# seceq/zkir

Hardware: AMD Instinct MI355X
Metric: trace rows/sec (2^20-cycle fib: execution-trace fill + BabyBear NTT/LDE + Poseidon2 Merkle commitment) (higher is better)
Workload: dtype u32 (Baby Bear, 31-bit modular) / u64 trace words

## Files before the change

include/zkir_amd_experimental.h:

```cpp
#ifndef ZKIR_AMD_EXPERIMENTAL_H
#define ZKIR_AMD_EXPERIMENTAL_H
#include "zkir_amd.h"
#ifdef __cplusplus
extern "C" {
#endif

double zkir_modmul_peak_per_s(void* hip_stream);
double zkir_hbm_copy_peak_gbs(uint64_t bytes, void* hip_stream);
int zkir_commit_fused01_launch(const zkir_stark_ctx* ctx, const zkir_trace_columns* trace, uint64_t n_real, uint32_t* m, uint32_t width, uint32_t* out, void* hip_stream);
int zkir_ntt_strided_variant_launch(const zkir_stark_ctx* ctx, uint32_t* data, uint32_t width, int variant, int forward, void* hip_stream);

int zkir_commit_overlapped_launch(const zkir_stark_ctx* ctx, uint32_t* in, uint32_t width, uint32_t* out, uint32_t* tree, uint32_t group, void* hip_stream);

int zkir_lowdeg_prove_stages(zkir_stark_ctx* ctx, const uint32_t* lde_mat, uint32_t width, const uint32_t* tree, uint32_t num_queries, uint32_t pow_bits, uint32_t* proof_host,
                             uint64_t cap_words, uint64_t* n_words, float stage_ms[4], void* hip_stream);
int zkir_lowdeg_combine_launch(const zkir_stark_ctx* ctx, const uint32_t* lde_mat, uint32_t width, const uint32_t gamma[4], uint32_t* gpow_scratch, uint32_t* cw, void* hip_stream);

int zkir_eval_prove_stages(zkir_stark_ctx* ctx, const uint32_t* lde_mat, uint32_t width, const uint32_t* tree, const uint32_t* points, uint32_t n_points, uint32_t num_queries,
                           uint32_t pow_bits, uint32_t* proof_host, uint64_t cap_words, uint64_t* n_words, float stage_ms[6], void* hip_stream);
uint64_t zkir_eval_at_scratch_words(uint32_t log_n, uint32_t width, uint32_t n_points);
int zkir_eval_at_launch(const zkir_stark_ctx* ctx, const uint32_t* lde_mat, uint32_t width, const uint32_t* points, uint32_t n_points, uint32_t* scratch, uint32_t* evals, void* hip_stream);
uint64_t zkir_eval_quotient_scratch_words(uint32_t log_m, uint32_t width, uint32_t n_points);
int zkir_eval_quotient_launch(const zkir_stark_ctx* ctx, const uint32_t* lde_mat, uint32_t width, const uint32_t gamma[4], const uint32_t* points, uint32_t n_points,
                              const uint32_t* evals, uint32_t* scratch, uint32_t* cw, void* hip_stream);
// ... 26 lines not shown
int zkir_verify_many_memory_probe(const uint32_t* const* proofs, const uint64_t* proof_words, const zkir_public_inputs* const* expects, uint32_t n, int32_t* verdicts, uint32_t what,
                                  uint32_t index, int device, void* hip_stream);
int zkir_verify_many_tapes_host(const uint32_t* const* proofs, const uint64_t* proof_words, const zkir_public_inputs* const* expects, uint32_t n, int32_t* verdicts);
int zkir_verify_rate_many_tapes_host(const uint32_t* const* proofs, const uint64_t* proof_words, const zkir_public_inputs* const* expects, const uint32_t* min_queries,
                                     const uint32_t* min_pow_bits, uint32_t n, int32_t* verdicts);
int zkir_tape_sections_stage_host(const uint32_t* const* hash_secs, const uint64_t* hash_words, const uint32_t* const* wide_secs, const uint64_t* wide_words, const uint64_t* n_real,
                                  const uint64_t* code_end, const uint32_t* alphas, const uint32_t* lambdas, uint32_t n, int32_t* hash_verdicts, int32_t* wide_verdicts, uint32_t* digests,
                                  uint32_t* sums);
int zkir_tape_sections_stage_launch(const uint32_t* const* hash_secs, const uint64_t* hash_words, const uint32_t* const* wide_secs, const uint64_t* wide_words, const uint64_t* n_real,
                                    const uint64_t* code_end, const uint32_t* alphas, const uint32_t* lambdas, uint32_t n, int32_t* hash_verdicts, int32_t* wide_verdicts, uint32_t* digests,
                                    uint32_t* sums, void* hip_stream);
int zkir_verify_many_tapes_probe(const uint32_t* const* proofs, const uint64_t* proof_words, const zkir_public_inputs* const* expects, uint32_t n, int32_t* verdicts, uint32_t what,
                                 uint32_t index, int device, void* hip_stream);
void zkir_poseidon2_scaled_quads(const uint32_t* in, uint64_t n, uint32_t* full, uint32_t* quads);
int zkir_poseidon2_sponge_full_blocks(const uint32_t* words, uint32_t n_words, uint32_t form, uint32_t digest[4]);

#ifdef __cplusplus
}
#endif
#endif
```

zkir_amd/csrc/host.h:

```cpp
#pragma once

#include <sys/mman.h>

#include <atomic>
#include <cstdint>
#include <cstdlib>
#include <cstring>
#include <new>
#include <string>
#include <utility>
#include <vector>

#include "../../include/zkir_amd.h"

#define ZKIR_DEFAULT_TILE_ROWS 1024u

namespace zkir {

struct Status {
  int code = ZKIR_OK;
  std::string msg;
  bool ok() const { return code == ZKIR_OK; }
};

// ... 142 lines not shown
                         void* hip_stream);

struct LdeTables {
  int log_n;
  const uint32_t* tw_inv;
  const uint32_t* tw_fwd;
  const uint32_t* g_lo;
  const uint32_t* g_hi;
  const uint32_t* small_inv;
  const uint32_t* small_fwd;
  int log_blowup = 1;
  uint32_t* zero_slot = nullptr;
  uint32_t zero_epoch = 0;
};
constexpr uint32_t ZERO_FLAG_BLOCKS = 64;
void lde_run(const LdeTables& t, uint32_t* in, uint32_t n_blocks, uint32_t* out, void* hip_stream);
bool strided_variant_run(const LdeTables& t, uint32_t* data, uint32_t n_blocks, int variant, bool dit, void* hip_stream);
bool lde_run_fused01(const LdeTables& t, const zkir_trace_columns* trace, uint64_t n_real, uint32_t* in, uint32_t n_blocks, uint32_t* out, void* hip_stream);
}
```

zkir_amd/csrc/ntt.hip:

```cpp
#include <hip/hip_runtime.h>

#include <atomic>
#include <cstdlib>
#include <mutex>
#include <type_traits>

#include "../../include/zkir_amd.h"
#include "../../include/zkir_amd_experimental.h"
#include "babybear.h"
#include "host.h"

namespace {

constexpr int NT = 256;
__device__ __forceinline__ uint32_t bitrev(uint32_t x, int bits) { return bits == 0 ? 0u : __brev(x) >> (32 - bits); }

template <int K, int N, class F>
__device__ __forceinline__ void static_for(F&& f) {
  if constexpr (K < N) { f(std::integral_constant<int, K>{}); static_for<K + 1, N>(f); }
}

using u32x4 = uint32_t __attribute__((ext_vector_type(4)));
__device__ __forceinline__ u32x4 ld4(const uint4* p) { return *reinterpret_cast<const u32x4*>(p); }
__device__ __forceinline__ void st4(uint4* p, u32x4 v) { *reinterpret_cast<u32x4*>(p) = v; }

__device__ __forceinline__ void wave_sync_lds() { asm volatile("s_waitcnt lgkmcnt(0)" ::: "memory"); }

struct WTw { int32_t w, n; };
__device__ __forceinline__ WTw wtw(int32_t w) { return WTw{w, -w}; }
__device__ __forceinline__ void dit4w4(uint4& x0, uint4& x1, uint4& x2, uint4& x3, WTw w1, WTw w2, WTw w2i) {
#define ZKIR_Q(c, e) { int32_t a[4] = {(int32_t)x0.c, (int32_t)x1.c, (int32_t)x2.c, (int32_t)x3.c}, b[4] = {(int32_t)x0.e, (int32_t)x1.e, (int32_t)x2.e, (int32_t)x3.e}; \
                       bb::dit4w2(a, b, w1.w, w1.n, w2.w, w2.n, w2i.w, w2i.n); \
                       x0.c = (uint32_t)a[0]; x1.c = (uint32_t)a[1]; x2.c = (uint32_t)a[2]; x3.c = (uint32_t)a[3]; x0.e = (uint32_t)b[0]; x1.e = (uint32_t)b[1]; x2.e = (uint32_t)b[2]; x3.e = (uint32_t)b[3]; }
  ZKIR_Q(x, y) __builtin_amdgcn_sched_barrier(0); ZKIR_Q(z, w)
#undef ZKIR_Q
// ... 50 lines not shown
      const uint64_t v = q.t.registers[o];
      const int bits = q.t.reg_state[o] ? 30 : 20;
      const uint64_t mask = (1ull << bits) - 1;
      out[0] = (uint32_t)(v & mask); out[1] = (uint32_t)((v >> bits) & mask); out[2] = (uint32_t)(v >> (2 * bits));
    };
    uint32_t a[3], b[3];
    if (half == 0) { limbs(1, a); r.x = q.t.instruction[src] >> 19; r.y = a[0]; r.z = a[1]; r.w = a[2]; }
    else { limbs(2, a); limbs(3, b); r.x = a[0]; r.y = a[1]; r.z = a[2]; r.w = b[0]; }
  }
  return r;
}

template <bool DIT, int R, int C, int NTH, bool FUSED = false>
__global__ __launch_bounds__(NTH) void ntt_strided_r4_kernel(uint4* __restrict__ data, uint64_t blk_u4, uint32_t tiles_per_block, uint32_t total, int L, int s0,
                                                              const uint32_t* __restrict__ tw, const uint32_t* __restrict__ small, int log_small, uint32_t j4_m, int canon, TraceSrc01 fsrc = TraceSrc01{},
                                                              uint32_t* zflags = nullptr, uint32_t epoch = 0, int produce = 0) {
  constexpr int B = 2 * R;
  constexpr uint32_t POS = 1u << (B + C), QUADS = POS / 4, CMASK = (1u << C) - 1, PLANE = POS + 4;
  constexpr uint32_t MOVES = 2 * POS / NTH;
  static_assert(QUADS % NTH == 0 && NTH % (1 << C) == 0 && (2 * POS) % NTH == 0, "tile / thread geometry");
  extern __shared__ uint4 lds4[];
  const uint32_t n = 1u << L;
  const uint32_t stride_mid = DIT ? (1u << s0) : (n >> (s0 + B));
  const uint32_t lo_tiles = stride_mid >> C;
  auto geometry = [&](uint32_t w, uint4*& x, uint32_t& base, uint32_t& lo0, uint32_t& hi) {
    const uint32_t tile = w % tiles_per_block;
    x = data + (uint64_t)(w / tiles_per_block) * blk_u4;
    hi = tile / lo_tiles;
    lo0 = (tile % lo_tiles) << C;
    base = (DIT ? (hi << (s0 + B)) : hi * (n >> s0)) + lo0;
  };
  static_assert(QUADS == NTH, "one quad per lane and round");
  u32x4 pre[MOVES];
  uint4* x; uint32_t base, lo0, hi;
  uint64_t live = ~0ull;
  if (zflags && !produce) { const uint32_t l = threadIdx.x & 63; live = __ballot(l < total / tiles_per_block && zflags[l] == epoch); }
  auto next_live = [&](uint32_t ww) { while (ww < total && !((live >> (ww / tiles_per_block)) & 1)) ww += gridDim.x; return ww; };
  uint32_t w = next_live(blockIdx.x);
  if (w >= total) return;
  uint32_t sm[R];
#pragma unroll
  for (int r = 0; r < R; r++) {
    const int b = 2 * r;
    const uint32_t qq = threadIdx.x >> C;
    if (!DIT) sm[r] = small[bitrev(qq >> (B - 2 - b), b) << (log_small - (b + 2))];
    else sm[r] = small[(qq & ((1u << b) - 1)) << (log_small - (b + 2))];
  }
  const bool unit = s0 == 0;
  uint32_t tf_next[R] = {};
  auto tile_factors = [&](uint32_t hi_t) {
    if (DIT || unit) return;
    const uint32_t e = bitrev(hi_t, s0);
#pragma unroll
    for (int r = 0; r < R; r++) tf_next[r] = tw[e << (L - s0 - 2 * r - 2)];
// ... 2 lines not shown
  static_for<0, (int)MOVES>([&](auto kc) {
    constexpr uint32_t k = decltype(kc)::value;
    const uint32_t e = threadIdx.x + k * NTH, row = e >> (C + 1), wv = e & ((2u << C) - 1);
    if constexpr (FUSED) pre[k] = trace_quad01(fsrc, w / tiles_per_block, wv & 1, (uint64_t)base + (uint64_t)row * stride_mid + (wv >> 1));
    else pre[k] = ld4(&x[((uint64_t)base + (uint64_t)row * stride_mid) * 2 + wv]);
  });
  uint32_t tw_cur = 0;
  if (DIT) tw_cur = tw[(lo0 + (threadIdx.x & CMASK)) << (L - s0 - B)];
  tile_factors(hi);
  for (;;) {
    uint32_t nz = 0;
    static_for<0, (int)MOVES>([&](auto kc) {
      constexpr uint32_t k = decltype(kc)::value;
      const uint32_t e = threadIdx.x + k * NTH, row = e >> (C + 1), wv = e & ((2u << C) - 1);
      st4(&lds4[(wv & 1) * PLANE + ((row << C) | (wv >> 1))], pre[k]);
      if (produce) nz |= (pre[k].x | pre[k].y) | (pre[k].z | pre[k].w);
    });
    uint32_t tp[R];
    if (DIT) {
      uint32_t u = tw_cur;
#pragma unroll
      for (int r = R - 1; r >= 0; r--) { tp[r] = u; u = bb::mont_mul(u, u); u = bb::mont_mul(u, u); }
    } else {
#pragma unroll
      for (int r = 0; r < R; r++) tp[r] = tf_next[r];
    }
    bool dense = true;
    if (produce) {
      dense = __syncthreads_or(nz != 0) != 0;
      if (dense && threadIdx.x == 0) zflags[w / tiles_per_block] = epoch;
    } else {
      __syncthreads();
    }
    const uint32_t wn = next_live(w + gridDim.x);
    uint4* xn = x; uint32_t base_n = base, lo0_n = lo0, hi_n = hi;
    if (wn < total) {
      geometry(wn, xn, base_n, lo0_n, hi_n);
      static_for<0, (int)MOVES>([&](auto kc) {
        constexpr uint32_t k = decltype(kc)::value;
        const uint32_t e = threadIdx.x + k * NTH, row = e >> (C + 1), wv = e & ((2u << C) - 1);
        if constexpr (FUSED) pre[k] = trace_quad01(fsrc, wn / tiles_per_block, wv & 1, (uint64_t)base_n + (uint64_t)row * stride_mid + (wv >> 1));
        else pre[k] = ld4(&xn[((uint64_t)base_n + (uint64_t)row * stride_mid) * 2 + wv]);
      });
      if (DIT) tw_cur = tw[(lo0_n + (threadIdx.x & CMASK)) << (L - s0 - B)];
      tile_factors(hi_n);
// ... 27 lines not shown
          const WTw w2 = wtw(bb::mont_mul_centred(tp[r], sm[r]));
          const uint32_t w2u = bb::wcanon(w2.w);
          const WTw w1 = wtw(bb::mont_mul_centred(w2u, w2u)), w2i = wtw(bb::mont_mul_centred(w2u, j4_m));
          uint4 x0 = pl0[i0], x1 = pl0[i0 + d], x2 = pl0[i0 + 2 * d], x3 = pl0[i0 + 3 * d];
          dit4w4(x0, x1, x2, x3, w1, w2, w2i);
          pl0[i0] = x0; pl0[i0 + d] = x1; pl0[i0 + 2 * d] = x2; pl0[i0 + 3 * d] = x3;
          __builtin_amdgcn_sched_barrier(0);
          uint4 y0 = pl1[i0], y1 = pl1[i0 + d], y2 = pl1[i0 + 2 * d], y3 = pl1[i0 + 3 * d];
          dit4w4(y0, y1, y2, y3, w1, w2, w2i);
          pl1[i0] = y0; pl1[i0 + d] = y1; pl1[i0 + 2 * d] = y2; pl1[i0 + 3 * d] = y3;
        }
      }
      const bool wave_local = !DIT ? (r + 1 < R && B - 2 - b <= 6 - C) : (r + 1 < R && b + 2 <= 6 - C);
      if (wave_local) wave_sync_lds(); else __syncthreads();
    }
#pragma unroll
    for (uint32_t k = 0; k < MOVES; k++) {
      const uint32_t e = threadIdx.x + k * NTH, row = e >> (C + 1), wv = e & ((2u << C) - 1);
      uint4 v = lds4[(wv & 1) * PLANE + ((row << C) | (wv >> 1))];
      if (DIT && canon) v = canon4(v);
      x[((uint64_t)base + (uint64_t)row * stride_mid) * 2 + wv] = v;
    }
    }
    if (wn >= total) break;
    w = wn; x = xn; base = base_n; lo0 = lo0_n; hi = hi_n;
  }
}

template <bool DIT, int S>
__global__ __launch_bounds__(NT) void ntt_reg_kernel(uint4* __restrict__ data, uint64_t blk_u4, int L, int s0, const uint32_t* __restrict__ tw, uint32_t r4_m, uint32_t r8_m,
                                                       uint32_t r8_3_m, int canon) {
  constexpr int E = 1 << S;
  const uint32_t n = 1u << L;
  uint4* x = data + (uint64_t)blockIdx.y * blk_u4;
  const uint64_t item = (uint64_t)blockIdx.x * NT + threadIdx.x;
  if (item >= ((uint64_t)n >> S) * 2) return;
// ... 40 lines not shown
}

inline unsigned cu_count() {
  static std::mutex mu;
  static unsigned cached[64] = {};
  int dev = 0;
  if (hipGetDevice(&dev) != hipSuccess || dev < 0 || dev >= 64) return 256u;
  std::lock_guard<std::mutex> lk(mu);
  if (!cached[dev]) { hipDeviceProp_t p; cached[dev] = hipGetDeviceProperties(&p, dev) == hipSuccess && p.multiProcessorCount > 0 ? (unsigned)p.multiProcessorCount : 256u; }
  return cached[dev];
}
inline int persist() { static const int v = getenv("ZKIR_NTT_PERSIST") ? atoi(getenv("ZKIR_NTT_PERSIST")) : 1; return v; }

template <bool DIT, int R, int C, int NTH, bool FUSED = false>
void launch_strided_r4(uint32_t* data, uint64_t n, uint32_t n_blocks, int L, int s0, const uint32_t* tw, const uint32_t* small, int log_small, uint32_t j4_m, hipStream_t s,
                       const TraceSrc01* fsrc = nullptr, int canon = 0, uint32_t* zflags = nullptr, uint32_t epoch = 0, int produce = 0) {
  constexpr size_t lds = 16u * 2 * ((1u << (2 * R + C)) + 4);
  auto k = ntt_strided_r4_kernel<DIT, R, C, NTH, FUSED>;
  static std::atomic<uint64_t> attr_done{0};
  int dev = 0; (void)hipGetDevice(&dev);
  const uint64_t bit = 1ull << (dev & 63);
  if (!(attr_done.load(std::memory_order_relaxed) & bit)) { (void)hipFuncSetAttribute(reinterpret_cast<const void*>(k), hipFuncAttributeMaxDynamicSharedMemorySize, (int)lds); attr_done.fetch_or(bit); }
  const uint32_t tiles = (uint32_t)(n >> (2 * R + C)), total = tiles * n_blocks;
  const unsigned per_cu = (unsigned)((160u << 10) / lds) > 0 ? (unsigned)((160u << 10) / lds) : 1u;
  unsigned grid = persist() ? cu_count() * (per_cu > 8 ? 8 : per_cu) : total;
  if (grid > total) grid = total;
  hipLaunchKernelGGL(k, dim3(grid), dim3(NTH), lds, s, (uint4*)data, 2 * n, tiles, total, L, s0, tw, small, log_small, j4_m, canon, fsrc ? *fsrc : TraceSrc01{}, zflags, epoch, produce);
}

inline int strided_c() { static const int c = getenv("ZKIR_NTT_C") ? atoi(getenv("ZKIR_NTT_C")) : 2; return c; }

template <bool DIT>
uint32_t* run_strided_stages(uint32_t* data, uint64_t n, uint32_t n_blocks, int L, int s0, int stages, const uint32_t* tw, const uint32_t* small, int log_small, uint32_t j4_m,
                             uint32_t r8_m, uint32_t r8_3_m, hipStream_t s, uint32_t* zflags = nullptr, uint32_t epoch = 0, bool produce = false) {
  bool first = true;
  while (stages > 0) {
    int take;
    if (stages >= 10 && stages != 11) take = 10;
    else if (stages == 11) take = 8;
    else if (stages == 9) take = 6;
    else if (stages == 7) take = 4;
    else if (stages == 5) take = 3;
    else take = stages;
    const int canon = DIT && take == stages;
    int pr = 0;
    if (produce && first) { if (take >= 4) pr = 1; else zflags = nullptr; }
    first = false;
    switch (take) {
      case 10:
        if (strided_c() == 2) launch_strided_r4<DIT, 5, 2, 1024>(data, n, n_blocks, L, s0, tw, small, log_small, j4_m, s, nullptr, canon, zflags, epoch, pr);
        else launch_strided_r4<DIT, 5, 1, 512>(data, n, n_blocks, L, s0, tw, small, log_small, j4_m, s, nullptr, canon, zflags, epoch, pr);
        break;
      case 8: launch_strided_r4<DIT, 4, 3, 512>(data, n, n_blocks, L, s0, tw, small, log_small, j4_m, s, nullptr, canon, zflags, epoch, pr); break;
      case 6: launch_strided_r4<DIT, 3, 4, 256>(data, n, n_blocks, L, s0, tw, small, log_small, j4_m, s, nullptr, canon, zflags, epoch, pr); break;
      case 4: launch_strided_r4<DIT, 2, 5, 128>(data, n, n_blocks, L, s0, tw, small, log_small, j4_m, s, nullptr, canon, zflags, epoch, pr); break;
      case 3:
        hipLaunchKernelGGL((ntt_reg_kernel<DIT, 3>), dim3((unsigned)(((n >> 3) * 2 + NT - 1) / NT), n_blocks), dim3(NT), 0, s, (uint4*)data, 2 * n, L, s0, tw, j4_m, r8_m, r8_3_m, canon);
        break;
      case 2:
        hipLaunchKernelGGL((ntt_reg_kernel<DIT, 2>), dim3((unsigned)(((n >> 2) * 2 + NT - 1) / NT), n_blocks), dim3(NT), 0, s, (uint4*)data, 2 * n, L, s0, tw, j4_m, r8_m, r8_3_m, canon);
        break;
      default:
        hipLaunchKernelGGL(ntt_stage_kernel<DIT>, dim3((unsigned)((n + NT - 1) / NT), n_blocks), dim3(NT), 0, s, (uint4*)data, 2 * n, L, s0, tw, canon);
        break;
    }
    s0 += take; stages -= take;
  }
  return zflags;
}

// ... 31 lines not shown
        const uint32_t ia = (r_hi << (s + 1)) | r_lo, ib = ia + half;
        const uint32_t a = lds[ia], t = bb::mont_mul(lds[ib], small_fwd[r_lo << (L - s)]);
        lds[ia] = bb::add(a, t); lds[ib] = bb::sub(a, t);
      }
      __syncthreads();
    }
    for (uint32_t e = threadIdx.x; e < 2 * n; e += NT) y[(uint64_t)e * 8 + c] = lds[e];
    __syncthreads();
  }
}

constexpr int MID_NT = 512;
__global__ __launch_bounds__(MID_NT) __attribute__((amdgpu_waves_per_eu(4, 4))) void lde_middle_r4_kernel(const uint4* __restrict__ in, uint4* __restrict__ out, uint32_t chunks_per_block, uint32_t total, int L,
                                                                const uint32_t* __restrict__ tw_inv, const uint32_t* __restrict__ small_inv, const uint32_t* __restrict__ small_fwd,
                                                                const uint32_t* __restrict__ g_lo, const uint32_t* __restrict__ g_hi, uint32_t j4_inv_m, uint32_t j4_fwd_m, int canon,
                                                                const uint32_t* __restrict__ zflags, uint32_t epoch) {
  constexpr int Bm = 10;
  constexpr uint32_t APL = 1024;
  __shared__ uint4 A[2 * APL];
  __shared__ uint4 Bf[2048];
  const uint32_t n = 1u << L, t = threadIdx.x;
  uint64_t live = ~0ull;
  if (zflags) { const uint32_t l = t & 63; live = __ballot(l < total / chunks_per_block && zflags[l] == epoch); }
  auto next_live = [&](uint32_t ww) {
    for (; ww < total && !((live >> (ww / chunks_per_block)) & 1); ww += gridDim.x) {
      uint4* yz = out + (uint64_t)(ww / chunks_per_block) * n * 4 + ((uint64_t)(ww % chunks_per_block) << (Bm + 2));
#pragma unroll
      for (int k = 0; k < 4; k++) { const uint32_t e = t + k * MID_NT; yz[2 * e] = make_uint4(0, 0, 0, 0); yz[2 * e + 1] = make_uint4(0, 0, 0, 0); }
    }
    return ww;
  };
  uint32_t w = next_live(blockIdx.x);
  if (w >= total) return;
  uint32_t tw_i[5], tw_f[5];
#pragma unroll
  for (int r = 0; r < 5; r++) {
    const int lg = 8 - 2 * r;
    tw_i[r] = small_inv[bitrev((t & 255) >> lg, 2 * r) << lg];
    const int sft = 2 * r + 1;
    tw_f[r] = small_fwd[(t & ((1u << sft) - 1)) << (Bm - sft - 1)];
  }
  u32x4 pre[4];
  uint32_t cf_next[5];
  uint32_t glo[4], ghi[4];
  auto fetch = [&](uint32_t ww) {
    const uint4* x = in + ((uint64_t)(ww / chunks_per_block) * n + ((uint64_t)(ww % chunks_per_block) << Bm)) * 2;
#pragma unroll
    for (int k = 0; k < 4; k++) pre[k] = ld4(&x[t + k * MID_NT]);
    const uint32_t p0 = ((ww % chunks_per_block) << Bm) + 4 * (t & 255);
#pragma unroll
    for (int i = 0; i < 4; i++) { const uint32_t k = bitrev(p0 + i, L); glo[i] = g_lo[k & 1023]; ghi[i] = g_hi[k >> 10]; }
    const uint32_t ce = bitrev(ww % chunks_per_block, L - Bm);
#pragma unroll
    for (int r = 0; r < 5; r++) cf_next[r] = tw_inv[ce << (8 - 2 * r)];
  };
  fetch(w);
  for (;;) {
    const uint32_t base = (w % chunks_per_block) << Bm;
    uint4* y = out + (uint64_t)(w / chunks_per_block) * n * 4;
#pragma unroll
    for (int k = 0; k < 4; k++) { const uint32_t e = t + k * MID_NT; st4(&A[(e & 1) * APL + (e >> 1)], pre[k]); }
    uint32_t gs[4];
#pragma unroll
// ... 222 lines not shown
    run_strided_stages<false>(in, N, n_blocks, L, 0, L - 10, t.tw_inv, t.small_inv, 10, j4_inv_m, r8_inv_m, r8_inv3_m, s);
    const uint32_t chunks = N >> 10, total = chunks * n_blocks;
    unsigned grid = persist() ? cu_count() * 2 : total;
    if (grid > total) grid = total;
    auto mid = LB == 2 ? lde_middle_blowup_kernel<2> : lde_middle_blowup_kernel<3>;
    hipLaunchKernelGGL(mid, dim3(grid), dim3(MID_NT), 0, s, (const uint4*)in, (uint4*)out, chunks, total, L, t.tw_inv, t.small_inv, t.small_fwd, t.g_lo, t.g_hi, j4_inv_m, j4_fwd_m, L == 10);
    run_strided_stages<true>(out, (uint64_t)N << LB, n_blocks, L + LB, 10 + LB, L - 10, t.tw_fwd, t.small_fwd, 10 + LB, j4_fwd_m, r8_fwd_m, r8_fwd3_m, s);
    return;
  }
  if (L < 10) {
    hipLaunchKernelGGL(lde_small_kernel, dim3(n_blocks), dim3(NT), (8u << L), s, in, out, L, t.small_inv, t.small_fwd, t.g_lo, t.g_hi);
    return;
  }
  uint32_t* zf = t.zero_slot && t.zero_epoch && n_blocks <= ZERO_FLAG_BLOCKS ? t.zero_slot : nullptr;
  zf = run_strided_stages<false>(in, N, n_blocks, L, 0, L - 10, t.tw_inv, t.small_inv, 10, j4_inv_m, r8_inv_m, r8_inv3_m, s, zf, t.zero_epoch, zf != nullptr);
  {
    const uint32_t chunks = N >> 10, total = chunks * n_blocks;
    unsigned grid = persist() ? cu_count() * 2 : total;
    if (grid > total) grid = total;
    hipLaunchKernelGGL(lde_middle_r4_kernel, dim3(grid), dim3(MID_NT), 0, s, (const uint4*)in, (uint4*)out, chunks, total, L, t.tw_inv, t.small_inv, t.small_fwd, t.g_lo, t.g_hi,
                       j4_inv_m, j4_fwd_m, L == 10, (const uint32_t*)zf, t.zero_epoch);
  }
  run_strided_stages<true>(out, (uint64_t)2 * N, n_blocks, L + 1, 11, L - 10, t.tw_fwd, t.small_fwd, 11, j4_fwd_m, r8_fwd_m, r8_fwd3_m, s, zf, t.zero_epoch);
}


bool strided_variant_run(const LdeTables& t, uint32_t* data, uint32_t n_blocks, int variant, bool dit, void* stream) {
  hipStream_t s = (hipStream_t)stream;
  const int L = dit ? t.log_n + 1 : t.log_n;
  if (t.log_n < 20) return false;
  const uint64_t n = (uint64_t)1 << L;
  static const uint32_t j4_inv_m = bb::to_mont(bb::inv(bb::root_of_unity(2))), j4_fwd_m = bb::to_mont(bb::root_of_unity(2));
  const uint32_t* tw = dit ? t.tw_fwd : t.tw_inv; const uint32_t* sm = dit ? t.small_fwd : t.small_inv;
  const int ls = dit ? 11 : 10; const uint32_t j4 = dit ? j4_fwd_m : j4_inv_m; const int s0 = dit ? 11 : 0;
#define ZKIR_VARIANT(R, C, NTH) do { if (dit) launch_strided_r4<true, R, C, NTH>(data, n, n_blocks, L, s0, tw, sm, ls, j4, s); else launch_strided_r4<false, R, C, NTH>(data, n, n_blocks, L, s0, tw, sm, ls, j4, s); } while (0)
  switch (variant) {
    case 0: ZKIR_VARIANT(5, 2, 1024); break;
    case 1: ZKIR_VARIANT(5, 1, 512); break;
// ... 12 lines not shown
  if (L < 20 || L == 21 || n_blocks < 3 || strided_c() != 2) return false;
  const uint32_t N = 1u << L;
  static const uint32_t j4_inv_m = bb::to_mont(bb::inv(bb::root_of_unity(2))), j4_fwd_m = bb::to_mont(bb::root_of_unity(2));
  static const uint32_t r8_fwd = bb::root_of_unity(3), r8_inv = bb::inv(r8_fwd);
  static const uint32_t r8_inv_m = bb::to_mont(r8_inv), r8_inv3_m = bb::to_mont(bb::mul(bb::mul(r8_inv, r8_inv), r8_inv));
  static const uint32_t r8_fwd_m = bb::to_mont(r8_fwd), r8_fwd3_m = bb::to_mont(bb::mul(bb::mul(r8_fwd, r8_fwd), r8_fwd));
  const TraceSrc01 src{*trace, n_real};
  launch_strided_r4<false, 5, 2, 1024, true>(in, N, 2, L, 0, t.tw_inv, t.small_inv, 10, j4_inv_m, s, &src);
  launch_strided_r4<false, 5, 2, 1024>(in + (uint64_t)2 * N * 8, N, n_blocks - 2, L, 0, t.tw_inv, t.small_inv, 10, j4_inv_m, s);
  if (L - 10 > 10) run_strided_stages<false>(in, N, n_blocks, L, 10, L - 20, t.tw_inv, t.small_inv, 10, j4_inv_m, r8_inv_m, r8_inv3_m, s);
  {
    const uint32_t chunks = N >> 10, total = chunks * n_blocks;
    unsigned grid = persist() ? cu_count() * 2 : total;
    if (grid > total) grid = total;
    hipLaunchKernelGGL(lde_middle_r4_kernel, dim3(grid), dim3(MID_NT), 0, s, (const uint4*)in, (uint4*)out, chunks, total, L, t.tw_inv, t.small_inv, t.small_fwd, t.g_lo, t.g_hi,
                       j4_inv_m, j4_fwd_m, L == 10, nullptr, 0u);
  }
  run_strided_stages<true>(out, (uint64_t)2 * N, n_blocks, L + 1, 11, L - 10, t.tw_fwd, t.small_fwd, 11, j4_fwd_m, r8_fwd_m, r8_fwd3_m, s);
  return true;
}

}
```

zkir_amd/csrc/stark.hip:

```cpp
#include <hip/hip_runtime.h>

#include <array>
#include <atomic>
#include <chrono>
#include <cstdio>
#include <cstdlib>
#include <cstddef>
#include <memory>
#include <mutex>
#include <vector>

#include "../../include/zkir_amd.h"
#include "../../include/zkir_amd_experimental.h"
#include "air.h"
#include "babybear.h"
#include "fri_shape.h"
#include "host.h"
#include "hashcall.h"
#include "poseidon2.h"
#include "verify_stages.h"

namespace {

constexpr int NT = 256;
// ... 614 lines not shown

constexpr uint32_t SYNC_SLOTS = 1024;
struct SyncRing {
  uint32_t* d_slots = nullptr;
  std::atomic<uint32_t> next{0};
  uint32_t* take() { return d_slots + (next.fetch_add(1, std::memory_order_relaxed) % SYNC_SLOTS); }
};

constexpr uint32_t ZERO_SLOTS = 1024;
struct ZeroFlagRing {
  uint32_t* d_words = nullptr;
  std::atomic<uint32_t> next{0};
  void take(uint32_t*& slot, uint32_t& epoch) {
    uint32_t e = next.fetch_add(1, std::memory_order_relaxed) + 1;
    if (e == 0) e = next.fetch_add(1, std::memory_order_relaxed) + 1;
    slot = d_words + (size_t)(e % ZERO_SLOTS) * zkir::ZERO_FLAG_BLOCKS; epoch = e;
  }
};

void launch_tree_levels(const p2::Consts* cp, uint32_t* leaf_digests, uint64_t n_leaves, SyncRing& ring, hipStream_t s) {
  uint32_t* cur = leaf_digests;
  uint64_t m = n_leaves;
  for (; m > (1u << 18); m >>= 1) {
    uint32_t* nxt = cur + 4 * m;
    hipLaunchKernelGGL(compress_kernel, dim3(grid_for(m / 2)), dim3(NT), 0, s, cp, cur, m / 2, nxt);
    cur = nxt;
  }
  if (m > 1) {
    const uint32_t per = m < SUBTREE ? (uint32_t)m : SUBTREE;
    hipLaunchKernelGGL(subtree_kernel, dim3((unsigned)(m / per)), dim3(NT_SUB), 0, s, cp, cur, m, per, ring.take());
  }
// ... 171 lines not shown
  c->log_n = log_n; c->log_blowup = log_blowup;
  const uint32_t N = 1u << log_n;
  const uint32_t n_inv = N >= 2 ? N / 2 : 1, n_hi = (N >> 10) + 1;
  const uint32_t n_fwd = N << (log_blowup - 1);
  p2::generate(c->consts);
  hipError_t e = hipMalloc((void**)&c->d_p2, sizeof(p2::Consts));
  if (e == hipSuccess) e = hipMemcpy(c->d_p2, &c->consts, sizeof(p2::Consts), hipMemcpyHostToDevice);
  for (int m = 0; m < 2 && e == hipSuccess; m++) {
    p2::Consts fwd;
    p2::generate(fwd, m ? bb::R1 : 1u);
    e = hipMalloc((void**)&c->d_p2_fwd[m], sizeof(p2::Consts));
    if (e == hipSuccess) e = hipMemcpy(c->d_p2_fwd[m], &fwd, sizeof(p2::Consts), hipMemcpyHostToDevice);
  }
  if (e == hipSuccess) e = hipMalloc(&c->sync.d_slots, SYNC_SLOTS * sizeof(uint32_t));
  if (e == hipSuccess) e = hipMemset(c->sync.d_slots, 0, SYNC_SLOTS * sizeof(uint32_t));
  if (e == hipSuccess) e = hipMalloc(&c->zero.d_words, (size_t)ZERO_SLOTS * zkir::ZERO_FLAG_BLOCKS * sizeof(uint32_t));
  if (e == hipSuccess) e = hipMemset(c->zero.d_words, 0, (size_t)ZERO_SLOTS * zkir::ZERO_FLAG_BLOCKS * sizeof(uint32_t));
  if (e == hipSuccess) e = hipMalloc(&c->d_tw_inv, (size_t)n_inv * 4);
  if (e == hipSuccess) e = hipMalloc(&c->d_tw_fwd, (size_t)n_fwd * 4);
  if (e == hipSuccess) e = hipMalloc(&c->d_g_lo, 1024 * 4);
  if (e == hipSuccess) e = hipMalloc(&c->d_g_hi, (size_t)n_hi * 4);
  if (e == hipSuccess) e = hipMalloc(&c->d_g_lo_m, 1024 * 4);
  if (e == hipSuccess && log_blowup == 1) e = hipMalloc(&c->d_inv_xm1, (size_t)2 * N * 4);
  const int Bm = log_n < 10 ? (int)log_n : 10;
  const uint32_t n_si = Bm >= 1 ? (1u << (Bm - 1)) : 1, n_sf = 1u << (Bm + log_blowup - 1);
  if (e == hipSuccess) e = hipMalloc(&c->d_small_inv, (size_t)n_si * 4);
  if (e == hipSuccess) e = hipMalloc(&c->d_small_fwd, (size_t)n_sf * 4);
  if (e != hipSuccess) { zkir::set_last_error({ZKIR_ERR_DEVICE, std::string("zkir_stark_ctx_create: ") + hipGetErrorString(e)}); zkir_stark_ctx_free(c); return ZKIR_ERR_DEVICE; }
  const uint32_t wN = bb::root_of_unity(log_n), wM = bb::root_of_unity(log_n + log_blowup);
  hipLaunchKernelGGL(powers_kernel, dim3(grid_for(n_inv)), dim3(NT), 0, 0, bb::inv(wN), bb::R1, c->d_tw_inv, n_inv);
  hipLaunchKernelGGL(powers_kernel, dim3(grid_for(n_fwd)), dim3(NT), 0, 0, wM, bb::R1, c->d_tw_fwd, n_fwd);
  hipLaunchKernelGGL(powers_kernel, dim3(4), dim3(NT), 0, 0, bb::GEN, bb::to_mont(bb::inv(N % bb::P)), c->d_g_lo, 1024u);
// ... 195 lines not shown
```

zkir_amd/runtime.py:

```python
from __future__ import annotations

import ctypes as C
import os
from dataclasses import dataclass
from typing import List, Optional, Sequence, Tuple

import numpy as np

from .spec import Program

_HERE = os.path.dirname(os.path.abspath(__file__))
_SO = os.environ.get("ZKIR_AMD_LIB") or os.path.join(_HERE, "libzkir_amd.so")

(ZKIR_OK, ERR_MISALIGNED, ERR_INVALID_MEMORY, ERR_DIV_ZERO, ERR_INVALID_SYSCALL, ERR_DECODE, ERR_OTHER, ERR_BAD_PROGRAM,
 ERR_DEVICE, ERR_ARGUMENT) = range(10)
HALT_EBREAK, HALT_EXIT, HALT_CYCLE_LIMIT = 0, 1, 2

REG_EVENT_DTYPE = np.dtype([("value", "<u8"), ("payload", "<u8"), ("max_bits", "<u4"), ("vis", "<u4"), ("reg", "u1"),
                            ("state", "u1"), ("tag", "u1"), ("pad", "u1", (5,))])
MEM_EVENT_DTYPE = np.dtype([("address", "<u8"), ("value", "<u8"), ("row", "<u4"), ("is_write", "u1"), ("width", "u1"), ("pad", "<u2")])
RC_EVENT_DTYPE = np.dtype([("value", "<u8"), ("pc", "<u8")])
NORM_EVENT_DTYPE = np.dtype([("cycle", "<u8"), ("pc", "<u8"), ("raw_value", "<u8"), ("reg", "u1"), ("state", "u1"), ("opcode", "u1"),
                             ("pad", "u1", (5,))])
SHA_BLOCK_DTYPE = np.dtype([("message_block", "<u4", (16,)), ("timestamp", "<u8")])
# ... 423 lines not shown
        L.zkir_verify_rate_chain_device.restype = C.c_int; L.zkir_verify_rate_chain_device.argtypes = [V, V, U32, C.POINTER(PublicInputsC), U32, U32, V]
        L.zkir_verify_rate_many_device.restype = C.c_int; L.zkir_verify_rate_many_device.argtypes = [V, V, V, V, V, U32, V, V]
        L.zkir_pcs_verify_many_device.restype = C.c_int; L.zkir_pcs_verify_many_device.argtypes = [V, V, V, V, V, V, U32, V, V]
    L.zkir_prove_result.restype = C.c_int
    L.zkir_prove_result.argtypes = [V, C.POINTER(ProverParamsC), C.POINTER(C.POINTER(C.c_uint8)), C.POINTER(C.c_size_t)]
    L.zkir_proof_bytes_free.restype = None
    L.zkir_proof_bytes_free.argtypes = [C.POINTER(C.c_uint8)]
    L.zkir_proof_free.restype = None
    L.zkir_proof_free.argtypes = [C.POINTER(C.c_uint32)]
    L.zkir_proof_num_queries.restype = U32
    L.zkir_poseidon2_permute.restype = None; L.zkir_poseidon2_permute.argtypes = [C.c_void_p]
    L.zkir_poseidon2_permute_scaled.restype = None; L.zkir_poseidon2_permute_scaled.argtypes = [C.c_void_p, C.c_uint32]
    if hasattr(L, "zkir_poseidon2_scaled_quads"):
        L.zkir_poseidon2_scaled_quads.restype = None; L.zkir_poseidon2_scaled_quads.argtypes = [C.c_void_p, C.c_uint64, C.c_void_p, C.c_void_p]
        L.zkir_poseidon2_sponge_full_blocks.restype = C.c_int; L.zkir_poseidon2_sponge_full_blocks.argtypes = [C.c_void_p, C.c_uint32, C.c_uint32, C.c_void_p]
    L.zkir_exec.restype = C.c_int
    L.zkir_exec.argtypes = [C.c_char_p, C.c_size_t, C.POINTER(C.c_uint64), C.c_size_t, C.POINTER(VmConfigC), C.POINTER(C.c_void_p)]
    L.zkir_result_free.argtypes = [C.c_void_p]
    L.zkir_result_free.restype = None
    L.zkir_result_delta_log.restype = C.c_void_p
    L.zkir_result_delta_log.argtypes = [C.c_void_p]
    L.zkir_result_trace.restype = C.POINTER(TraceColumnsC)
    L.zkir_result_trace.argtypes = [C.c_void_p]
    L.zkir_result_stage_ms.restype = None
    L.zkir_result_stage_ms.argtypes = [C.c_void_p, C.POINTER(C.c_float)]
    L.zkir_result_copy_column.restype = C.c_int
    L.zkir_result_copy_column.argtypes = [C.c_void_p, C.c_int, C.c_int, C.c_void_p]
    for name, st in [("memory_trace", MemoryWitnessC), ("range_check_witnesses", RangeCheckWitnessC),
                     ("normalization_witnesses", NormalizationWitnessC), ("sha256_witnesses", Sha256WitnessC)]:
        f = getattr(L, "zkir_result_" + name)
# ... 878 lines not shown
```

Measured before the change: 203.0 million.

## Track zero flags per plane and pack half-live LDE columns in pairs

Zero-column tracking now keeps two flags per column block, one for each interleaved plane, so a block whose data lives in only one plane is recognised. The middle LDE kernel and the first DIT strided pass pair two such half-live blocks, so one tile's work serves both, and scatter the results back to their planes with zeros written into the dead plane. The goal is to cut NTT arithmetic and LDS traffic for sparse trace columns. It adds ballot and LDS bookkeeping in the producer pass, a doubled flag buffer, and fairly intricate pairing index math that could be wrong.

After: 209.0 million (median of 6 runs). 1.03x the previous value.

```diff
diff --git a/include/zkir_amd_experimental.h b/include/zkir_amd_experimental.h
--- a/include/zkir_amd_experimental.h
+++ b/include/zkir_amd_experimental.h
@@ -64,6 +64,7 @@
                                  uint32_t index, int device, void* hip_stream);
 void zkir_poseidon2_scaled_quads(const uint32_t* in, uint64_t n, uint32_t* full, uint32_t* quads);
 int zkir_poseidon2_sponge_full_blocks(const uint32_t* words, uint32_t n_words, uint32_t form, uint32_t digest[4]);
+uint32_t zkir_lde_plane_pairs(uint64_t live0, uint64_t live1, uint32_t* entries);
 
 #ifdef __cplusplus
 }
diff --git a/zkir_amd/csrc/host.h b/zkir_amd/csrc/host.h
--- a/zkir_amd/csrc/host.h
+++ b/zkir_amd/csrc/host.h
@@ -180,6 +180,7 @@
   uint32_t zero_epoch = 0;
 };
 constexpr uint32_t ZERO_FLAG_BLOCKS = 64;
+constexpr uint32_t ZERO_FLAG_WORDS = 2 * ZERO_FLAG_BLOCKS;
 void lde_run(const LdeTables& t, uint32_t* in, uint32_t n_blocks, uint32_t* out, void* hip_stream);
 bool strided_variant_run(const LdeTables& t, uint32_t* data, uint32_t n_blocks, int variant, bool dit, void* hip_stream);
 bool lde_run_fused01(const LdeTables& t, const zkir_trace_columns* trace, uint64_t n_real, uint32_t* in, uint32_t n_blocks, uint32_t* out, void* hip_stream);
diff --git a/zkir_amd/csrc/ntt.hip b/zkir_amd/csrc/ntt.hip
--- a/zkir_amd/csrc/ntt.hip
+++ b/zkir_amd/csrc/ntt.hip
@@ -19,6 +19,17 @@
 __device__ __forceinline__ void static_for(F&& f) {
   if constexpr (K < N) { f(std::integral_constant<int, K>{}); static_for<K + 1, N>(f); }
 }
+
+struct PlanePairs { uint64_t first, second; };
+BB_HD PlanePairs plane_pairs(uint64_t live0, uint64_t live1) {
+  const uint64_t half = live0 ^ live1;
+  uint64_t odd = half;
+  odd ^= odd << 1; odd ^= odd << 2; odd ^= odd << 4; odd ^= odd << 8; odd ^= odd << 16; odd ^= odd << 32;
+  uint64_t first = half & odd;
+  if (__builtin_popcountll(half) & 1) first &= ~(1ull << (63 - __builtin_clzll(half)));
+  return PlanePairs{first, half & ~odd};
+}
+BB_HD uint32_t pair_partner(uint64_t second, uint32_t a) { return (uint32_t)__builtin_ctzll(second & ~((2ull << a) - 1)); }
 
 using u32x4 = uint32_t __attribute__((ext_vector_type(4)));
 __device__ __forceinline__ u32x4 ld4(const uint4* p) { return *reinterpret_cast<const u32x4*>(p); }
@@ -99,7 +110,7 @@
 template <bool DIT, int R, int C, int NTH, bool FUSED = false>
 __global__ __launch_bounds__(NTH) void ntt_strided_r4_kernel(uint4* __restrict__ data, uint64_t blk_u4, uint32_t tiles_per_block, uint32_t total, int L, int s0,
                                                               const uint32_t* __restrict__ tw, const uint32_t* __restrict__ small, int log_small, uint32_t j4_m, int canon, TraceSrc01 fsrc = TraceSrc01{},
-                                                              uint32_t* zflags = nullptr, uint32_t epoch = 0, int produce = 0) {
+                                                              uint32_t* zflags = nullptr, uint32_t epoch = 0, int produce = 0, int pack = 0) {
   constexpr int B = 2 * R;
   constexpr uint32_t POS = 1u << (B + C), QUADS = POS / 4, CMASK = (1u << C) - 1, PLANE = POS + 4;
   constexpr uint32_t MOVES = 2 * POS / NTH;
@@ -116,13 +127,25 @@
     base = (DIT ? (hi << (s0 + B)) : hi * (n >> s0)) + lo0;
   };
   static_assert(QUADS == NTH, "one quad per lane and round");
+  constexpr bool PACKS = DIT && !FUSED && ((R == 5 && C == 2) || (R == 4 && C == 3) || (R == 3 && C == 4) || (R == 2 && C == 5));
   u32x4 pre[MOVES];
   uint4* x; uint32_t base, lo0, hi;
-  uint64_t live = ~0ull;
-  if (zflags && !produce) { const uint32_t l = threadIdx.x & 63; live = __ballot(l < total / tiles_per_block && zflags[l] == epoch); }
+  uint64_t live = ~0ull, pair_a = 0, pair_b = 0, live1 = 0;
+  if (zflags && !produce) {
+    const uint32_t l = threadIdx.x & 63;
+    const bool in = l < total / tiles_per_block;
+    const uint64_t m0 = __ballot(in && zflags[2 * l] == epoch), m1 = __ballot(in && zflags[2 * l + 1] == epoch);
+    live = m0 | m1;
+    if constexpr (PACKS) {
+      if (pack) { const PlanePairs pp = plane_pairs(m0, m1); pair_a = pp.first; pair_b = pp.second; live1 = m1; live &= ~pair_b; }
+    }
+  }
   auto next_live = [&](uint32_t ww) { while (ww < total && !((live >> (ww / tiles_per_block)) & 1)) ww += gridDim.x; return ww; };
   uint32_t w = next_live(blockIdx.x);
   if (w >= total) return;
+  uint32_t* const tile_seen = reinterpret_cast<uint32_t*>(&lds4[POS]);
+  uint32_t seq = 1;
+  if (!DIT && produce) { if (threadIdx.x == 0) { tile_seen[0] = 0; tile_seen[1] = 0; } __syncthreads(); }
   uint32_t sm[R];
 #pragma unroll
   for (int r = 0; r < R; r++) {
@@ -155,7 +178,7 @@
       constexpr uint32_t k = decltype(kc)::value;
       const uint32_t e = threadIdx.x + k * NTH, row = e >> (C + 1), wv = e & ((2u << C) - 1);
       st4(&lds4[(wv & 1) * PLANE + ((row << C) | (wv >> 1))], pre[k]);
-      if (produce) nz |= (pre[k].x | pre[k].y) | (pre[k].z | pre[k].w);
+      if (!DIT && produce) nz |= (pre[k].x | pre[k].y) | (pre[k].z | pre[k].w);
     });
     uint32_t tp[R];
     if (DIT) {
@@ -167,9 +190,21 @@
       for (int r = 0; r < R; r++) tp[r] = tf_next[r];
     }
     bool dense = true;
-    if (produce) {
-      dense = __syncthreads_or(nz != 0) != 0;
-      if (dense && threadIdx.x == 0) zflags[w / tiles_per_block] = epoch;
+    if (!DIT && produce) {
+      const uint64_t bal = __ballot(nz != 0);
+      if ((threadIdx.x & 63) == 0) {
+        if (bal & 0x5555555555555555ull) tile_seen[0] = seq;
+        if (bal & 0xAAAAAAAAAAAAAAAAull) tile_seen[1] = seq;
+      }
+      __syncthreads();
+      const bool p0 = tile_seen[0] == seq, p1 = tile_seen[1] == seq;
+      dense = p0 || p1;
+      if (threadIdx.x == 0) {
+        const uint32_t blk = w / tiles_per_block;
+        if (p0) zflags[2 * blk] = epoch;
+        if (p1) zflags[2 * blk + 1] = epoch;
+      }
+      seq++;
     } else {
       __syncthreads();
     }
@@ -227,12 +262,30 @@
       const bool wave_local = !DIT ? (r + 1 < R && B - 2 - b <= 6 - C) : (r + 1 < R && b + 2 <= 6 - C);
       if (wave_local) wave_sync_lds(); else __syncthreads();
     }
+    bool paired = false;
+    if constexpr (PACKS) paired = (pair_a >> (w / tiles_per_block)) & 1;
+    if (PACKS && paired) {
+      const uint32_t ba = w / tiles_per_block, bp = pair_partner(pair_b, ba);
+      const uint32_t plane_a = (uint32_t)(live1 >> ba) & 1, plane_b = (uint32_t)(live1 >> bp) & 1;
+      const bool odd = threadIdx.x & 1;
+      uint4* xd = x + (odd ? (uint64_t)(bp - ba) * blk_u4 : 0);
+      const uint32_t plane = odd ? plane_b : plane_a;
+#pragma unroll
+      for (uint32_t k = 0; k < MOVES; k++) {
+        const uint32_t e = threadIdx.x + k * NTH, row = e >> (C + 1), wv = e & ((2u << C) - 1);
+        uint4 v = lds4[(wv & 1) * PLANE + ((row << C) | (wv >> 1))];
+        if (canon) v = canon4(v);
+        const uint64_t at = ((uint64_t)base + (uint64_t)row * stride_mid) * 2 + (wv & ~1u);
+        xd[at + plane] = v; xd[at + (plane ^ 1)] = make_uint4(0, 0, 0, 0);
+      }
+    } else {
 #pragma unroll
     for (uint32_t k = 0; k < MOVES; k++) {
       const uint32_t e = threadIdx.x + k * NTH, row = e >> (C + 1), wv = e & ((2u << C) - 1);
       uint4 v = lds4[(wv & 1) * PLANE + ((row << C) | (wv >> 1))];
       if (DIT && canon) v = canon4(v);
       x[((uint64_t)base + (uint64_t)row * stride_mid) * 2 + wv] = v;
+    }
     }
     }
     if (wn >= total) break;
@@ -303,7 +356,7 @@
 
 template <bool DIT, int R, int C, int NTH, bool FUSED = false>
 void launch_strided_r4(uint32_t* data, uint64_t n, uint32_t n_blocks, int L, int s0, const uint32_t* tw, const uint32_t* small, int log_small, uint32_t j4_m, hipStream_t s,
-                       const TraceSrc01* fsrc = nullptr, int canon = 0, uint32_t* zflags = nullptr, uint32_t epoch = 0, int produce = 0) {
+                       const TraceSrc01* fsrc = nullptr, int canon = 0, uint32_t* zflags = nullptr, uint32_t epoch = 0, int produce = 0, int pack = 0) {
   constexpr size_t lds = 16u * 2 * ((1u << (2 * R + C)) + 4);
   auto k = ntt_strided_r4_kernel<DIT, R, C, NTH, FUSED>;
   static std::atomic<uint64_t> attr_done{0};
@@ -314,14 +367,15 @@
   const unsigned per_cu = (unsigned)((160u << 10) / lds) > 0 ? (unsigned)((160u << 10) / lds) : 1u;
   unsigned grid = persist() ? cu_count() * (per_cu > 8 ? 8 : per_cu) : total;
   if (grid > total) grid = total;
-  hipLaunchKernelGGL(k, dim3(grid), dim3(NTH), lds, s, (uint4*)data, 2 * n, tiles, total, L, s0, tw, small, log_small, j4_m, canon, fsrc ? *fsrc : TraceSrc01{}, zflags, epoch, produce);
+  hipLaunchKernelGGL(k, dim3(grid), dim3(NTH), lds, s, (uint4*)data, 2 * n, tiles, total, L, s0, tw, small, log_small, j4_m, canon, fsrc ? *fsrc : TraceSrc01{}, zflags, epoch, produce, pack);
 }
 
 inline int strided_c() { static const int c = getenv("ZKIR_NTT_C") ? atoi(getenv("ZKIR_NTT_C")) : 2; return c; }
+inline bool one_lds_pass(int stages) { return (stages == 10 && strided_c() == 2) || stages == 8 || stages == 6 || stages == 4; }
 
 template <bool DIT>
 uint32_t* run_strided_stages(uint32_t* data, uint64_t n, uint32_t n_blocks, int L, int s0, int stages, const uint32_t* tw, const uint32_t* small, int log_small, uint32_t j4_m,
-                             uint32_t r8_m, uint32_t r8_3_m, hipStream_t s, uint32_t* zflags = nullptr, uint32_t epoch = 0, bool produce = false) {
+                             uint32_t r8_m, uint32_t r8_3_m, hipStream_t s, uint32_t* zflags = nullptr, uint32_t epoch = 0, bool produce = false, bool pack = false) {
   bool first = true;
   while (stages > 0) {
     int take;
@@ -334,15 +388,16 @@
     const int canon = DIT && take == stages;
     int pr = 0;
     if (produce && first) { if (take >= 4) pr = 1; else zflags = nullptr; }
+    const int pk = pack && zflags && first && one_lds_pass(stages);
     first = false;
     switch (take) {
       case 10:
-        if (strided_c() == 2) launch_strided_r4<DIT, 5, 2, 1024>(data, n, n_blocks, L, s0, tw, small, log_small, j4_m, s, nullptr, canon, zflags, epoch, pr);
-        else launch_strided_r4<DIT, 5, 1, 512>(data, n, n_blocks, L, s0, tw, small, log_small, j4_m, s, nullptr, canon, zflags, epoch, pr);
+        if (strided_c() == 2) launch_strided_r4<DIT, 5, 2, 1024>(data, n, n_blocks, L, s0, tw, small, log_small, j4_m, s, nullptr, canon, zflags, epoch, pr, pk);
+        else launch_strided_r4<DIT, 5, 1, 512>(data, n, n_blocks, L, s0, tw, small, log_small, j4_m, s, nullptr, canon, zflags, epoch, pr, pk);
         break;
-      case 8: launch_strided_r4<DIT, 4, 3, 512>(data, n, n_blocks, L, s0, tw, small, log_small, j4_m, s, nullptr, canon, zflags, epoch, pr); break;
-      case 6: launch_strided_r4<DIT, 3, 4, 256>(data, n, n_blocks, L, s0, tw, small, log_small, j4_m, s, nullptr, canon, zflags, epoch, pr); break;
-      case 4: launch_strided_r4<DIT, 2, 5, 128>(data, n, n_blocks, L, s0, tw, small, log_small, j4_m, s, nullptr, canon, zflags, epoch, pr); break;
+      case 8: launch_strided_r4<DIT, 4, 3, 512>(data, n, n_blocks, L, s0, tw, small, log_small, j4_m, s, nullptr, canon, zflags, epoch, pr, pk); break;
+      case 6: launch_strided_r4<DIT, 3, 4, 256>(data, n, n_blocks, L, s0, tw, small, log_small, j4_m, s, nullptr, canon, zflags, epoch, pr, pk); break;
+      case 4: launch_strided_r4<DIT, 2, 5, 128>(data, n, n_blocks, L, s0, tw, small, log_small, j4_m, s, nullptr, canon, zflags, epoch, pr, pk); break;
       case 3:
         hipLaunchKernelGGL((ntt_reg_kernel<DIT, 3>), dim3((unsigned)(((n >> 3) * 2 + NT - 1) / NT), n_blocks), dim3(NT), 0, s, (uint4*)data, 2 * n, L, s0, tw, j4_m, r8_m, r8_3_m, canon);
         break;
@@ -404,16 +459,24 @@
 __global__ __launch_bounds__(MID_NT) __attribute__((amdgpu_waves_per_eu(4, 4))) void lde_middle_r4_kernel(const uint4* __restrict__ in, uint4* __restrict__ out, uint32_t chunks_per_block, uint32_t total, int L,
                                                                 const uint32_t* __restrict__ tw_inv, const uint32_t* __restrict__ small_inv, const uint32_t* __restrict__ small_fwd,
                                                                 const uint32_t* __restrict__ g_lo, const uint32_t* __restrict__ g_hi, uint32_t j4_inv_m, uint32_t j4_fwd_m, int canon,
-                                                                const uint32_t* __restrict__ zflags, uint32_t epoch) {
+                                                                const uint32_t* __restrict__ zflags, uint32_t epoch, int pack) {
   constexpr int Bm = 10;
   constexpr uint32_t APL = 1024;
   __shared__ uint4 A[2 * APL];
   __shared__ uint4 Bf[2048];
   const uint32_t n = 1u << L, t = threadIdx.x;
-  uint64_t live = ~0ull;
-  if (zflags) { const uint32_t l = t & 63; live = __ballot(l < total / chunks_per_block && zflags[l] == epoch); }
+  uint64_t live = ~0ull, pair_a = 0, pair_b = 0, live1 = 0;
+  if (zflags) {
+    const uint32_t l = t & 63;
+    const bool inside = l < total / chunks_per_block;
+    const uint64_t m0 = __ballot(inside && zflags[2 * l] == epoch), m1 = __ballot(inside && zflags[2 * l + 1] == epoch);
+    live = m0 | m1;
+    if (pack) { const PlanePairs pp = plane_pairs(m0, m1); pair_a = pp.first; pair_b = pp.second; live1 = m1; }
+  }
+  const uint64_t work = live & ~pair_b;
   auto next_live = [&](uint32_t ww) {
-    for (; ww < total && !((live >> (ww / chunks_per_block)) & 1); ww += gridDim.x) {
+    for (; ww < total && !((work >> (ww / chunks_per_block)) & 1); ww += gridDim.x) {
+      if ((pair_b >> (ww / chunks_per_block)) & 1) continue;
       uint4* yz = out + (uint64_t)(ww / chunks_per_block) * n * 4 + ((uint64_t)(ww % chunks_per_block) << (Bm + 2));
 #pragma unroll
       for (int k = 0; k < 4; k++) { const uint32_t e = t + k * MID_NT; yz[2 * e] = make_uint4(0, 0, 0, 0); yz[2 * e + 1] = make_uint4(0, 0, 0, 0); }
@@ -434,9 +497,16 @@
   uint32_t cf_next[5];
   uint32_t glo[4], ghi[4];
   auto fetch = [&](uint32_t ww) {
-    const uint4* x = in + ((uint64_t)(ww / chunks_per_block) * n + ((uint64_t)(ww % chunks_per_block) << Bm)) * 2;
-#pragma unroll
-    for (int k = 0; k < 4; k++) pre[k] = ld4(&x[t + k * MID_NT]);
+    const uint32_t blk = ww / chunks_per_block;
+    const uint4* x = in + ((uint64_t)blk * n + ((uint64_t)(ww % chunks_per_block) << Bm)) * 2;
+    uint32_t at = t;
+    if ((pair_a >> blk) & 1) {
+      const uint32_t bp = pair_partner(pair_b, blk);
+      const uint32_t plane_a = (uint32_t)(live1 >> blk) & 1, plane_b = (uint32_t)(live1 >> bp) & 1;
+      at = (t & ~1u) + ((t & 1) ? (bp - blk) * (n * 2) + plane_b : plane_a);
+    }
+#pragma unroll
+    for (int k = 0; k < 4; k++) pre[k] = ld4(&x[at + k * MID_NT]);
     const uint32_t p0 = ((ww % chunks_per_block) << Bm) + 4 * (t & 255);
 #pragma unroll
     for (int i = 0; i < 4; i++) { const uint32_t k = bitrev(p0 + i, L); glo[i] = g_lo[k & 1023]; ghi[i] = g_hi[k >> 10]; }
@@ -689,14 +759,15 @@
   }
   uint32_t* zf = t.zero_slot && t.zero_epoch && n_blocks <= ZERO_FLAG_BLOCKS ? t.zero_slot : nullptr;
   zf = run_strided_stages<false>(in, N, n_blocks, L, 0, L - 10, t.tw_inv, t.small_inv, 10, j4_inv_m, r8_inv_m, r8_inv3_m, s, zf, t.zero_epoch, zf != nullptr);
+  const bool pack = zf != nullptr && one_lds_pass(L - 10);
   {
     const uint32_t chunks = N >> 10, total = chunks * n_blocks;
     unsigned grid = persist() ? cu_count() * 2 : total;
     if (grid > total) grid = total;
     hipLaunchKernelGGL(lde_middle_r4_kernel, dim3(grid), dim3(MID_NT), 0, s, (const uint4*)in, (uint4*)out, chunks, total, L, t.tw_inv, t.small_inv, t.small_fwd, t.g_lo, t.g_hi,
-                       j4_inv_m, j4_fwd_m, L == 10, (const uint32_t*)zf, t.zero_epoch);
-  }
-  run_strided_stages<true>(out, (uint64_t)2 * N, n_blocks, L + 1, 11, L - 10, t.tw_fwd, t.small_fwd, 11, j4_fwd_m, r8_fwd_m, r8_fwd3_m, s, zf, t.zero_epoch);
+                       j4_inv_m, j4_fwd_m, L == 10, (const uint32_t*)zf, t.zero_epoch, (int)pack);
+  }
+  run_strided_stages<true>(out, (uint64_t)2 * N, n_blocks, L + 1, 11, L - 10, t.tw_fwd, t.small_fwd, 11, j4_fwd_m, r8_fwd_m, r8_fwd3_m, s, zf, t.zero_epoch, false, pack);
 }
 
 
@@ -739,10 +810,27 @@
     unsigned grid = persist() ? cu_count() * 2 : total;
     if (grid > total) grid = total;
     hipLaunchKernelGGL(lde_middle_r4_kernel, dim3(grid), dim3(MID_NT), 0, s, (const uint4*)in, (uint4*)out, chunks, total, L, t.tw_inv, t.small_inv, t.small_fwd, t.g_lo, t.g_hi,
-                       j4_inv_m, j4_fwd_m, L == 10, nullptr, 0u);
+                       j4_inv_m, j4_fwd_m, L == 10, nullptr, 0u, 0);
   }
   run_strided_stages<true>(out, (uint64_t)2 * N, n_blocks, L + 1, 11, L - 10, t.tw_fwd, t.small_fwd, 11, j4_fwd_m, r8_fwd_m, r8_fwd3_m, s);
   return true;
 }
 
 }
+
+extern "C" uint32_t zkir_lde_plane_pairs(uint64_t live0, uint64_t live1, uint32_t* entries) {
+  const PlanePairs pp = plane_pairs(live0, live1);
+  const uint64_t work = (live0 | live1) & ~pp.second;
+  uint32_t count = 0;
+  for (uint32_t b = 0; b < 64; b++) {
+    if (!((work >> b) & 1)) continue;
+    uint32_t* e = entries + 4 * count++;
+    if ((pp.first >> b) & 1) {
+      const uint32_t bp = pair_partner(pp.second, b);
+      e[0] = b; e[1] = (uint32_t)(live1 >> b) & 1; e[2] = bp; e[3] = (uint32_t)(live1 >> bp) & 1;
+    } else {
+      e[0] = b; e[1] = 2; e[2] = 0xFFFFFFFFu; e[3] = 2;
+    }
+  }
+  return count;
+}
diff --git a/zkir_amd/csrc/stark.hip b/zkir_amd/csrc/stark.hip
--- a/zkir_amd/csrc/stark.hip
+++ b/zkir_amd/csrc/stark.hip
@@ -652,7 +652,7 @@
   void take(uint32_t*& slot, uint32_t& epoch) {
     uint32_t e = next.fetch_add(1, std::memory_order_relaxed) + 1;
     if (e == 0) e = next.fetch_add(1, std::memory_order_relaxed) + 1;
-    slot = d_words + (size_t)(e % ZERO_SLOTS) * zkir::ZERO_FLAG_BLOCKS; epoch = e;
+    slot = d_words + (size_t)(e % ZERO_SLOTS) * zkir::ZERO_FLAG_WORDS; epoch = e;
   }
 };
 
@@ -854,8 +854,8 @@
   }
   if (e == hipSuccess) e = hipMalloc(&c->sync.d_slots, SYNC_SLOTS * sizeof(uint32_t));
   if (e == hipSuccess) e = hipMemset(c->sync.d_slots, 0, SYNC_SLOTS * sizeof(uint32_t));
-  if (e == hipSuccess) e = hipMalloc(&c->zero.d_words, (size_t)ZERO_SLOTS * zkir::ZERO_FLAG_BLOCKS * sizeof(uint32_t));
-  if (e == hipSuccess) e = hipMemset(c->zero.d_words, 0, (size_t)ZERO_SLOTS * zkir::ZERO_FLAG_BLOCKS * sizeof(uint32_t));
+  if (e == hipSuccess) e = hipMalloc(&c->zero.d_words, (size_t)ZERO_SLOTS * zkir::ZERO_FLAG_WORDS * sizeof(uint32_t));
+  if (e == hipSuccess) e = hipMemset(c->zero.d_words, 0, (size_t)ZERO_SLOTS * zkir::ZERO_FLAG_WORDS * sizeof(uint32_t));
   if (e == hipSuccess) e = hipMalloc(&c->d_tw_inv, (size_t)n_inv * 4);
   if (e == hipSuccess) e = hipMalloc(&c->d_tw_fwd, (size_t)n_fwd * 4);
   if (e == hipSuccess) e = hipMalloc(&c->d_g_lo, 1024 * 4);
diff --git a/zkir_amd/runtime.py b/zkir_amd/runtime.py
--- a/zkir_amd/runtime.py
+++ b/zkir_amd/runtime.py
@@ -461,6 +461,8 @@
     if hasattr(L, "zkir_poseidon2_scaled_quads"):
         L.zkir_poseidon2_scaled_quads.restype = None; L.zkir_poseidon2_scaled_quads.argtypes = [C.c_void_p, C.c_uint64, C.c_void_p, C.c_void_p]
         L.zkir_poseidon2_sponge_full_blocks.restype = C.c_int; L.zkir_poseidon2_sponge_full_blocks.argtypes = [C.c_void_p, C.c_uint32, C.c_uint32, C.c_void_p]
+    if hasattr(L, "zkir_lde_plane_pairs"):
+        L.zkir_lde_plane_pairs.restype = C.c_uint32; L.zkir_lde_plane_pairs.argtypes = [C.c_uint64, C.c_uint64, C.c_void_p]
     L.zkir_exec.restype = C.c_int
     L.zkir_exec.argtypes = [C.c_char_p, C.c_size_t, C.POINTER(C.c_uint64), C.c_size_t, C.POINTER(VmConfigC), C.POINTER(C.c_void_p)]
     L.zkir_result_free.argtypes = [C.c_void_p]
```
